# davidesantangelo/krep

Hardware: AMD Instinct MI355X
Metric: GB/s scanned (literal scan, match offsets produced), haystack resident in HBM (higher is better)
Workload: dtype u8; 1 GPU; literal8: 8-byte case-sensitive literal 'Sherlock', ~1e-4 matches/byte, offsets tracked; 32 GiB per GPU (BASELINE.json configs[1]); pattern=Sherlock, bytes_per_gpu=34359738368, matches=3436005, parallelism=contiguous shards x1, start-offset ownership, 1 RCCL all-reduce of counts

## Files before the change

include/krep_gpu_debug.h:

```cpp
#ifndef KREP_GPU_DEBUG_H
#define KREP_GPU_DEBUG_H
#include "krep_gpu.h"
#ifdef __cplusplus
extern "C" {
#endif

uint64_t krep_gpu_debug_replay_host(int krep_ref_algo, const void *text, size_t n, const void *pattern, uint32_t m,
                                    int whole_word, size_t cur, int open_line);
void krep_gpu_debug_force_rounds(int rounds);
void krep_gpu_debug_force_stage_cap(int records);
void krep_gpu_debug_force_single_grid(int blocks);
uint64_t krep_gpu_debug_single_failovers(void);
uint64_t krep_gpu_debug_single_launches(void);
uint64_t krep_gpu_debug_tiny_launches(void);
uint64_t krep_gpu_debug_tiny_dense_launches(void);
void krep_gpu_debug_inject_failure(int kind);
void krep_gpu_debug_chain_fixups(uint64_t *rescans, uint64_t *replays);
void krep_gpu_debug_fold_carry(const krep_gpu_seq_carry_t *in, const krep_gpu_seq_carry_t *piece, krep_gpu_seq_carry_t *out);
uint64_t krep_gpu_debug_anchored_launches(void);
uint64_t krep_gpu_debug_literal_dma_launches(void);
int krep_gpu_debug_literal_dma_state(const krep_gpu_plan_t *plan, int *looked, int *barred, double *pass_rate);
uint64_t krep_gpu_debug_runs_launches(void);
int krep_gpu_debug_split_state(const krep_gpu_plan_t *plan);
int krep_gpu_debug_anchor_info(const krep_gpu_plan_t *plan, int *state, uint32_t *moved, double *rate_end_grams, double *rate_anchors);
int krep_gpu_debug_anchor_measured(const krep_gpu_plan_t *plan, double *measured, int *resamples);

#ifdef __cplusplus
}
#endif
#endif
```

krep_amd/csrc/kg_config.hip:

```cpp
#include <hip/hip_runtime.h>

#include <algorithm>
#include <atomic>
#include <chrono>
#include <cstdarg>
#include <cstdio>
#include <cstdlib>
#include <cstring>
#include <mutex>
#include <string>
#include <vector>

#include "../../include/krep_gpu.h"
#include "kg_common.h"
#include "kg_internal.h"
#include "kg_plan.h"
#include "kg_replay.h"

using namespace kg;

static thread_local std::string g_err;
namespace kg {
int fail(const char *fmt, ...)
{
// ... 194 lines not shown
    const char *r = kg::device_unusable(kg::current_config().device);
    return r ? r : "";
}

namespace kg {
std::atomic<int> g_force_rounds{0};
std::atomic<int> g_force_stage_cap{0};
}
extern "C" void krep_gpu_debug_force_stage_cap(int c) { g_force_stage_cap.store(c); }
extern "C" void krep_gpu_debug_force_rounds(int r) { g_force_rounds.store(r); }
namespace kg {
extern int g_s1_force_grid;
std::atomic<uint64_t> g_fused1_failovers{0};
}
extern "C" void krep_gpu_debug_force_single_grid(int blocks) { kg::g_s1_force_grid = blocks < 0 ? 0 : blocks; }
extern "C" uint64_t krep_gpu_debug_single_failovers(void) { return g_fused1_failovers.load(); }
namespace kg {
std::atomic<uint64_t> g_fused1_launches{0};
}
extern "C" uint64_t krep_gpu_debug_single_launches(void) { return kg::g_fused1_launches.load(); }
namespace kg {
std::atomic<uint64_t> g_tiny_launches{0};
}
extern "C" uint64_t krep_gpu_debug_tiny_launches(void) { return kg::g_tiny_launches.load(); }
namespace kg {
std::atomic<uint64_t> g_tiny_dense_launches{0};
}
extern "C" uint64_t krep_gpu_debug_tiny_dense_launches(void) { return kg::g_tiny_dense_launches.load(); }
namespace kg {
std::atomic<uint64_t> g_ac_anchored_launches{0};
}
extern "C" uint64_t krep_gpu_debug_anchored_launches(void) { return kg::g_ac_anchored_launches.load(); }
extern "C" uint64_t krep_gpu_debug_literal_dma_launches(void) { return kg::g_lit_dma_launches.load(); }
extern "C" uint64_t krep_gpu_debug_runs_launches(void) { return kg::g_runs_launches.load(); }
```

krep_amd/csrc/kg_internal.h:

```cpp
#pragma once
#include <hip/hip_runtime.h>

#include <atomic>
#include <cstring>
#include <initializer_list>
#include <vector>

#include "../../include/krep_gpu.h"
#include "../../include/krep_gpu_debug.h"
#include "kg_common.h"

namespace kg {

int fail(const char *fmt, ...);
const char *device_unusable(int device);
bool inject(int kind);
#define HIPCHK(x)                                                                                 \
    do                                                                                            \
    {                                                                                             \
        hipError_t e_ = (x);                                                                      \
        if (e_ != hipSuccess)                                                                     \
            return kg::fail("%s failed: %s (%s:%d)", #x, hipGetErrorString(e_), __FILE__, __LINE__); \
    } while (0)

// ... 22 lines not shown
}

template <auto Kernel> hipError_t grant_dynamic_lds(int bytes)
{
    static std::atomic<bool> granted[64];
    int dev = 0;
    (void)hipGetDevice(&dev);
    const bool known = dev >= 0 && dev < 64;
    if (known && granted[dev].load(std::memory_order_acquire))
        return hipSuccess;
    const hipError_t e = hipFuncSetAttribute(reinterpret_cast<const void *>(Kernel), hipFuncAttributeMaxDynamicSharedMemorySize, bytes);
    if (e == hipSuccess && known)
        granted[dev].store(true, std::memory_order_release);
    return e;
}

hipError_t launch_literal(const LitArgs &a, uint32_t num_cu, hipStream_t st);
int runs_count_greedy(const uint8_t *d_text, uint64_t text_len, uint64_t lo, uint64_t hi, uint32_t m, uint8_t byte, bool ci, int num_cu,
                      unsigned long long *d_slots, unsigned long long *h_slots, hipStream_t st, uint64_t *total, uint64_t *end_p1);
bool literal_dma_eligible(const LitArgs &a);
hipError_t launch_literal_dma(const LitArgs &a, uint32_t num_cu, hipStream_t st);
hipError_t launch_dma_byte_look(const uint8_t *text, uint64_t lo, uint32_t n_cells, uint32_t prefilter, bool ci, unsigned long long *out, hipStream_t st);
extern std::atomic<uint64_t> g_runs_launches;
extern std::atomic<uint64_t> g_lit_dma_launches;

struct PostScratch;
constexpr int kFusedShapeMax = 5;
double single_fused_max_density(int shape);
int single_fused_shape_for(double density, double margin, int start);
bool single_fused_reopens(uint64_t total, uint64_t span);
constexpr int kFusedGaveUp = 1;
int single_fused_run(const LitArgs &a, uint64_t n_units, uint64_t span, PostScratch &post, Counters *d_ctr, Counters *h_ctr,
                     uint32_t num_cu, int *shape, hipEvent_t ev_end, hipStream_t st, bool count_launch);

struct PostScratch
{
    unsigned long long *d_unitinfo = nullptr;
    unsigned long long *d_offsets = nullptr;
    unsigned long long *d_blk = nullptr;
    uint64_t units_cap = 0;
    unsigned long long *d_stage = nullptr;
    uint64_t stage_cap_words = 0;
    uint64_t *d_occ = nullptr;
    uint64_t occ_cap = 0;
    uint8_t *d_keep = nullptr;
    unsigned long long *d_gblk = nullptr;
    unsigned long long *d_surv = nullptr;
    uint64_t keep_cap = 0;
    unsigned long long *d_tk = nullptr;
    uint64_t tk_cap = 0;
};
void post_free(PostScratch &s);
int post_reserve(PostScratch &s, uint64_t n_units, uint64_t stage_words);
int post_order(PostScratch &s, uint64_t n_units, uint32_t stage_cap, uint32_t fixed_len, uint64_t origin, uint64_t unit_bytes,
               bool want_lines, uint64_t *d_pos, uint64_t pos_cap, Counters *d_ctr, int num_cu, hipStream_t st);
int post_offsets_pass(PostScratch &s, uint64_t n_units, bool want_lines, Counters *d_ctr, hipStream_t st);
int post_gather_pass(PostScratch &s, uint64_t n_units, uint32_t stage_cap, uint32_t fixed_len, uint64_t origin,
                     uint64_t unit_bytes, uint64_t *d_pos, uint64_t pos_cap, int num_cu, hipStream_t st);
constexpr uint32_t kWalkGreedy = 0;
constexpr uint32_t kWalkShortO = 1;
constexpr uint32_t kWalkShortOLines = 2;
struct WalkSpec
{
    uint32_t mode, m;
    bool ww, lines, ci;
    uint8_t b1, b2;
// ... 95 lines not shown
```

krep_amd/csrc/kg_literal_dma.hip:

```cpp
#include <hip/hip_runtime.h>
#include <algorithm>
#include <atomic>
#include <cstdlib>
#include "kg_common.h"
#include "kg_device.h"
#include "kg_internal.h"

namespace kg {

namespace {

constexpr u32 kDmaPark = 80;
constexpr u32 kDmaRing = 2u * kSegBytes;
constexpr u32 kDmaTail = 256u;
constexpr u32 kDmaWaveLds = kDmaRing + kDmaTail;
}

template <int KIND, bool MASKED, bool CI>
__global__ __launch_bounds__(kBlock, 2) void lit_scan_dma(const LitArgs a)
{
    extern __shared__ __attribute__((aligned(16))) uint8_t d_smem[];
    __shared__ u64 s_info_all[kWavesPerBlk][kDmaPark];
    __shared__ __attribute__((aligned(16))) unsigned short s_slots_all[kWavesPerBlk][kDmaPark * 16u];
    __shared__ u32 s_unit_all[kWavesPerBlk][kDmaPark];
    const u32 lane = lane_id();
    const u32 wave = __builtin_amdgcn_readfirstlane(threadIdx.x >> 6);
    uint8_t *ring = d_smem + wave * kDmaWaveLds;
    uint8_t *tailb = ring + kDmaRing;
    u64 *s_info = s_info_all[wave];
    unsigned short *s_slots = s_slots_all[wave];
    u32 *s_unit = s_unit_all[wave];
    const u32 ring_lds = (u32)(size_t)(__attribute__((address_space(3))) uint8_t *)ring;

    const bool want_pos = (a.flags & F_POS) != 0;
    const bool ww = (a.flags & F_WW) != 0;
    const u64 hi_match = (a.own_hi < a.text_len - a.m + 1) ? a.own_hi : (a.text_len - a.m + 1);
    constexpr u64 kUnitBytes = (u64)kRoundsBig * kSegBytes;
    const u64 n_units = a.num_tiles * kWavesPerBlk;

    const bool park = want_pos && a.stage_cap >= 16u && a.stage_cap <= 128u && (a.stage_cap & 7u) == 0u && n_units < (1ull << 32);
    const u32 park_max = park ? kDmaPark * 16u / a.stage_cap : 0u;
    u32 n_park = 0;
    auto flush_parked = [&]() __attribute__((always_inline)) {
        for (u32 i = lane; i < n_park; i += 64u)
        {
            const u64 u = s_unit[i];
            a.unitinfo[u] = s_info[i];
            if (s_info[i] & kUiCountMask)
            {
                uint4 *dst = reinterpret_cast<uint4 *>(reinterpret_cast<unsigned short *>(a.stage) + u * (u64)a.stage_cap);
                const uint4 *src = reinterpret_cast<const uint4 *>(&s_slots[i * a.stage_cap]);
                const u32 c = (u32)(s_info[i] & kUiCountMask), nv = ((c < a.stage_cap ? c : a.stage_cap) + 7u) >> 3;
                for (u32 q = 0; q < nv; ++q)
                    dst[q] = src[q];
            }
        }
        n_park = 0;
    };

    const u32 tk_units = a.upt ? a.upt : 1u;
    u64 static_next = (u64)blockIdx.x * kWavesPerBlk + wave;
    auto next_ticket = [&]() -> u64 {
        if (a.upt)
        {
            return wave_fetch_add(&a.ctr->ticket, 1ull, lane) * (u64)a.upt;
        }
        const u64 u = static_next;
        static_next += (u64)gridDim.x * kWavesPerBlk;
        return u;
    };
    auto issue_round = [&](u64 seg, u32 buf) -> bool {
        if (seg + kSegBytes > a.text_len)
            return false;
        const uint8_t *src = a.text + seg + lane * 16u;
        uint8_t *dst = ring + buf * kSegBytes;
#pragma unroll
        for (int j = 0; j < kCells; ++j)
            __builtin_amdgcn_global_load_lds((const __attribute__((address_space(1))) void *)(src + j * kCellBytes),
                                             (__attribute__((address_space(3))) void *)(dst + j * kCellBytes), 16, 0, 2 );
        return true;
    };
    auto issue_tail = [&](u64 at) -> bool {
        if (at + kDmaTail > a.text_len)
            return false;
        __builtin_amdgcn_global_load_lds((const __attribute__((address_space(1))) void *)(a.text + at + lane * 4u),
                                         (__attribute__((address_space(3))) void *)tailb, 4, 0, 0);
        return true;
    };

    u64 acc_total = 0;
    u32 pf_cells = 0;
    u32 wcnt = 0;
    auto stage_hit = [&](u64 unit, u32 idx, u32 rel) __attribute__((always_inline)) {
        if (idx < a.stage_cap)
        {
            unsigned short *slot = park ? &s_slots[n_park * a.stage_cap] : reinterpret_cast<unsigned short *>(a.stage) + unit * (u64)a.stage_cap;
            slot[idx] = (unsigned short)rel;
        }
    };
    auto publish = [&](u64 unit) __attribute__((always_inline)) {
        acc_total += wcnt;
        if (want_pos)
        {
            if (lane == 0)
            {
                const u64 info = (u64)wcnt | (wcnt ? (kLnHead | kLnTail) : 0ull);
                if (park)
                {
                    s_info[n_park] = info;
                    s_unit[n_park] = (u32)unit;
                }
                else
                    a.unitinfo[unit] = info;
                if (wcnt > a.stage_cap)
                {
                    atomicAdd(&a.ctr->overflow_units, 1ull);
                    atomicMax(&a.ctr->max_unit_count, (u64)wcnt);
                }
            }
            if (park && ++n_park == park_max)
                flush_parked();
        }
        wcnt = 0;
    };
    auto exact = [&](u32 A0, u32 A4) -> bool {
        const u32 e0 = CI ? (A0 | a.l0) : A0;
        bool h = (KIND == 4 && MASKED) ? (((e0 ^ a.p0) & a.k0) == 0u) : (e0 == a.p0);
        if (KIND >= 8)
        {
            const u32 e4 = CI ? (A4 | a.l1) : A4;
            h = h && ((KIND == 8 && MASKED) ? (((e4 ^ a.p1) & a.k1) == 0u) : (e4 == a.p1));
        }
        return h;
    };
    auto owned = [&](u64 p) -> bool { return p >= a.own_lo && p < hi_match && !(p >= a.excl_lo && p < a.excl_hi); };
    auto word_ok = [&](u64 p) -> bool {
        if (p > 0 && p != a.ww_exempt_left && is_wordc(a.text[p - 1]))
            return false;
        if (p + a.m < a.text_len && is_wordc(a.text[p + a.m]))
            return false;
        return true;
    };
    auto boundary = [&](u64 seg_prev, u64 unit, u32 r_prev, u32 c0, u32 c1, u32 n0, u32 n1) __attribute__((always_inline)) {
        {
            const u32 f = 0x01010101u * ((CI ? (a.p0 | 0x20u) : a.p0) & 0xffu);
            const u32 y0 = (CI ? (c0 | 0x20202020u) : c0) ^ f, y1 = (CI ? (c1 | 0x20202020u) : c1) ^ f;
            if (((((y0 - 0x01010101u) & ~y0) | ((y1 - 0x01010101u) & ~y1)) & 0x80808080u) == 0u)
                return;
        }
        const u32 q = lane & 7u, sh = q & 3u;
        const bool up = (q >> 2) != 0u;
        const u32 lo = up ? c1 : c0, mid = up ? n0 : c1, hi = up ? n1 : n0;
        const u32 A0 = __builtin_amdgcn_alignbyte(mid, lo, sh), A4 = __builtin_amdgcn_alignbyte(hi, mid, sh);
        const u64 p = seg_prev + (kSegBytes - 8u) + q;
        bool h = lane < 8u && q + a.m > 8u && exact(A0, A4) && owned(p);
        if (ww && __ballot(h))
            h = h && word_ok(p);
        const u64 bm = __ballot(h);
        if (bm)
        {
            if (h && want_pos)
                stage_hit(unit, wcnt + mbcnt64(bm), r_prev * kSegBytes + (kSegBytes - 8u) + q);
            wcnt += (u32)__popcll(bm);
        }
    };

    u64 u0 = next_ticket();
    bool dma_cur = u0 < n_units && issue_round(a.anchor + u0 * kUnitBytes, 0u);
    while (u0 < n_units)
    {
        const u32 nun = (u32)((n_units - u0 < (u64)tk_units) ? (n_units - u0) : (u64)tk_units), nr = nun * (u32)kRoundsBig;
        const u64 tbase = a.anchor + u0 * kUnitBytes;
        u64 u_next = ~0ull;
        bool tail_ok = false;
        u32 c0 = 0, c1 = 0;
        bool deferred = false;
#pragma unroll 1
        for (u32 g = 0; g < nr; ++g)
        {
            const u64 seg = tbase + (u64)g * kSegBytes, unit = u0 + (g >> 2);
            const u32 r = g & 3u;
            bool dma_nx = false, tail_now = false;
            asm volatile("s_waitcnt lgkmcnt(0)" ::: "memory");
            if (g + 1u < nr)
                dma_nx = issue_round(seg + kSegBytes, (g + 1u) & 1u);
            else
            {
                u_next = next_ticket();
                if (u_next < n_units)
                    dma_nx = issue_round(a.anchor + u_next * kUnitBytes, (g + 1u) & 1u);
            }
            if (g + 2u == nr)
                tail_ok = tail_now = issue_tail(tbase + (u64)nr * kSegBytes);
            if (dma_cur)
            {
                if (dma_nx && tail_now)
                    asm volatile("s_waitcnt vmcnt(9)" ::: "memory");
                else if (dma_nx)
                    asm volatile("s_waitcnt vmcnt(8)" ::: "memory");
                else if (tail_now)
                    asm volatile("s_waitcnt vmcnt(1)" ::: "memory");
                else
                    asm volatile("s_waitcnt vmcnt(0)" ::: "memory");
            }
            const bool interior = seg >= a.own_lo && seg + kSegBytes <= hi_match && (seg + kSegBytes <= a.excl_lo || seg >= a.excl_hi);
            uint4 vv[kCells];
            uint2 nn[kCells];
            if (dma_cur)
            {
                typedef u32 v4 __attribute__((ext_vector_type(4)));
                typedef u32 v2 __attribute__((ext_vector_type(2)));
                const u32 addr = ring_lds + (g & 1u) * kSegBytes + lane * 16u;
                v4 x[kCells];
                v2 y[kCells];
#pragma unroll
                for (int j = 0; j < kCells; ++j)
                {
                    asm volatile("ds_read_b128 %0, %1 offset:%2" : "=v"(x[j]) : "v"(addr), "n"(j * (int)kCellBytes));
                    asm volatile("ds_read_b64 %0, %1 offset:%2" : "=v"(y[j]) : "v"(addr), "n"(j * (int)kCellBytes + 16));
                }
                asm volatile("s_waitcnt lgkmcnt(0)"
                             : "+v"(x[0]), "+v"(x[1]), "+v"(x[2]), "+v"(x[3]), "+v"(x[4]), "+v"(x[5]), "+v"(x[6]), "+v"(x[7]), "+v"(y[0]), "+v"(y[1]),
                               "+v"(y[2]), "+v"(y[3]), "+v"(y[4]), "+v"(y[5]), "+v"(y[6]), "+v"(y[7])
                             :
                             : "memory");
#pragma unroll
                for (int j = 0; j < kCells; ++j)
                {
                    vv[j] = make_uint4(x[j].x, x[j].y, x[j].z, x[j].w);
                    nn[j] = make_uint2(y[j].x, y[j].y);
                }
            }
            else
            {
#pragma unroll
                for (int j = 0; j < kCells; ++j)
                {
                    const W6 w = load_window_guarded(a.text, a.text_len, seg + (u64)j * kCellBytes + (u64)lane * 16u);
                    vv[j] = make_uint4(w.v[0], w.v[1], w.v[2], w.v[3]);
                    nn[j] = make_uint2(w.v[4], w.v[5]);
                }
            }
            if (deferred)
            {
                boundary(seg - kSegBytes, u0 + ((g - 1u) >> 2), (g - 1u) & 3u, c0, c1, __builtin_amdgcn_readfirstlane(vv[0].x),
                         __builtin_amdgcn_readfirstlane(vv[0].y));
                deferred = false;
                if (r == 0u)
                    publish(unit - 1u);
            }
            __builtin_amdgcn_sched_barrier(0);
#pragma unroll
            for (int j = 0; j < kCells; ++j)
            {
                const u64 lbase = seg + (u64)j * kCellBytes + (u64)lane * 16u;
                const u32 D[6] = {vv[j].x, vv[j].y, vv[j].z, vv[j].w, nn[j].x, nn[j].y};
                auto A = [&](int k) -> u32 {
                    return ((k & 3) == 0) ? D[k >> 2] : __builtin_amdgcn_alignbyte(D[(k >> 2) + 1], D[k >> 2], (u32)(k & 3));
                };
                u32 Dq[6];
#pragma unroll
                for (int w = 0; w < 6; ++w)
                    Dq[w] = CI ? (D[w] | 0x20202020u) : D[w];
                auto Aq = [&](int k) -> u32 {
                    return ((k & 3) == 0) ? Dq[k >> 2] : __builtin_amdgcn_alignbyte(Dq[(k >> 2) + 1], Dq[k >> 2], (u32)(k & 3));
                };
                const u32 p0q = CI ? (a.p0 | 0x20202020u) : a.p0;
                if (a.prefilter)
                {
                    u32 z = 0;
#pragma unroll
                    for (int w = 0; w < 4; ++w)
                    {
                        const u32 y = Dq[w] ^ a.prefilter;
                        z |= (y - 0x01010101u) & ~y;
                    }
                    if (!__ballot((z & 0x80808080u) != 0u))
                        continue;
                    ++pf_cells;
                }
                bool c[16];
                u64 any = 0;
#pragma unroll
// ... 75 lines not shown
                    }
                }
            }
            if (dma_cur)
            {
                c0 = __builtin_amdgcn_readlane(vv[kCells - 1].z, 63);
                c1 = __builtin_amdgcn_readlane(vv[kCells - 1].w, 63);
                deferred = true;
            }
            if (g + 1u == nr)
            {
                if (deferred)
                {
                    u32 n0 = 0, n1 = 0;
                    if (tail_ok)
                    {
                        typedef u32 v2 __attribute__((ext_vector_type(2)));
                        v2 t;
                        const u32 taddr = ring_lds + kDmaRing;
                        asm volatile("ds_read_b64 %0, %1\n\ts_waitcnt lgkmcnt(0)" : "=v"(t) : "v"(taddr) : "memory");
                        n0 = __builtin_amdgcn_readfirstlane(t.x);
                        n1 = __builtin_amdgcn_readfirstlane(t.y);
                    }
                    else
                    {
                        const W6 w = load_window_guarded(a.text, a.text_len, seg + kSegBytes);
                        n0 = __builtin_amdgcn_readfirstlane(w.v[0]);
                        n1 = __builtin_amdgcn_readfirstlane(w.v[1]);
                    }
                    boundary(seg, unit, r, c0, c1, n0, n1);
                    deferred = false;
                }
                publish(unit);
            }
            else if (!deferred && r == 3u)
                publish(unit);
            dma_cur = dma_nx;
        }
        u0 = u_next;
    }
    if (park && n_park)
        flush_parked();
    if (lane == 0 && acc_total)
        atomicAdd(&a.ctr->total, acc_total);
    if (lane == 0 && pf_cells)
        atomicAdd(&a.ctr->candidates, (u64)pf_cells);
}

__global__ __launch_bounds__(256) void dma_byte_look(const uint8_t *text, u64 lo, u32 n_cells, u32 b4, u32 fold, unsigned long long *out)
{
    const u32 lane = lane_id();
    const u32 wave = blockIdx.x * 4u + (threadIdx.x >> 6), n_waves = gridDim.x * 4u;
    u32 cnt = 0;
    for (u32 c = wave; c < n_cells; c += n_waves)
    {
        const uint4 v = *reinterpret_cast<const uint4 *>(text + lo + (u64)c * kCellBytes + lane * 16u);
        const u32 d[4] = {v.x, v.y, v.z, v.w};
        u32 z = 0;
#pragma unroll
        for (int w = 0; w < 4; ++w)
        {
            const u32 y = (d[w] | fold) ^ b4;
            z |= (y - 0x01010101u) & ~y;
        }
        if (__ballot((z & 0x80808080u) != 0u))
            ++cnt;
    }
    if (lane == 0 && cnt)
        atomicAdd(out, (u64)cnt);
}
hipError_t launch_dma_byte_look(const uint8_t *text, uint64_t lo, uint32_t n_cells, uint32_t prefilter, bool ci, unsigned long long *out, hipStream_t st)
{
    hipLaunchKernelGGL(dma_byte_look, dim3(256), dim3(256), 0, st, text, (u64)lo, n_cells, prefilter, ci ? 0x20202020u : 0u, out);
    return hipGetLastError();
}

std::atomic<uint64_t> g_lit_dma_launches{0};

template <int KIND, bool MASKED, bool CI>
static hipError_t dma_launch3(const LitArgs &a, u32 num_cu, hipStream_t st)
{
    constexpr u32 lds = kWavesPerBlk * kDmaWaveLds;
    if (const hipError_t e = grant_dynamic_lds<&lit_scan_dma<KIND, MASKED, CI>>((int)lds); e != hipSuccess)
        return e;
    static const u32 bpc = [] { const char *e = getenv("KREP_GPU_LIT_DMA_BLOCKS_PER_CU"); return e && atoi(e) > 0 ? (u32)atoi(e) : 2u; }();
    const u32 grid = (u32)std::min<u64>(a.num_tiles, (u64)num_cu * bpc);
    hipLaunchKernelGGL((lit_scan_dma<KIND, MASKED, CI>), dim3(grid ? grid : 1), dim3(kBlock), lds, st, a);
    g_lit_dma_launches.fetch_add(1, std::memory_order_relaxed);
    return hipGetLastError();
}
template <int KIND, bool MASKED>
static hipError_t dma_launch2(const LitArgs &a, u32 num_cu, hipStream_t st)
{
    return (a.flags & F_CI) ? dma_launch3<KIND, MASKED, true>(a, num_cu, st) : dma_launch3<KIND, MASKED, false>(a, num_cu, st);
}

bool literal_dma_eligible(const LitArgs &a)
{
    return !getenv("KREP_GPU_LIT_NO_DMA") && a.prefilter != 0u && a.m >= 2 && a.m <= 8 && a.rounds == (u32)kRoundsBig && !(a.flags & F_LINES) && !a.emit_mode &&
           (a.upt >= 4 || getenv("KREP_GPU_LIT_DMA_ALL")) && a.text_len >= 4u * kSegBytes;
}
hipError_t launch_literal_dma(const LitArgs &a, u32 num_cu, hipStream_t st)
{
    if (a.m < 4)
        return dma_launch2<4, true>(a, num_cu, st);
    if (a.m == 4)
        return dma_launch2<4, false>(a, num_cu, st);
    if (a.m < 8)
        return dma_launch2<8, true>(a, num_cu, st);
    return dma_launch2<8, false>(a, num_cu, st);
}

}
```

krep_amd/csrc/kg_plan.h:

```cpp
#pragma once
#include <hip/hip_runtime.h>

#include <vector>

#include "../../include/krep_gpu.h"
#include "kg_common.h"
#include "kg_internal.h"

struct krep_gpu_plan
{
    krep_gpu_config_t cfg{};
    int device = 0;
    int ref_algo = KREP_RA_NONE;
    const char *unsupported = nullptr;
    bool only_matching = false;
    bool cs = true, ww = false, lines = false, track = false;
    size_t max_count = SIZE_MAX;
    std::vector<std::vector<uint8_t>> pats;
    uint32_t m = 0, p0 = 0, p1 = 0, k0 = 0, k1 = 0, l0 = 0, l1 = 0;
    uint32_t p2 = 0, p3 = 0, k2 = 0, k3 = 0, l2 = 0, l3 = 0;
    std::vector<uint8_t> pat_folded;
    bool has_border = false;
    bool has_newline = false;
    uint8_t *d_pat = nullptr;
    unsigned long long *d_pat_chunks = nullptr;
    uint32_t n_chunks = 0;
    kg::Counters *d_ctr = nullptr, *h_ctr = nullptr;
    int num_cu = 256;
    hipEvent_t ev0 = nullptr, ev1 = nullptr;
    kg::AcTables *ac = nullptr;
    kg::AcTables *ac_long = nullptr, *ac_short = nullptr;
    int ac_split = 0;
    match_position_t *d_split_rec = nullptr;
    uint64_t split_cap = 0;
    bool ac_has_newline = false;
    kg::PostScratch post;
    uint32_t sparse_cap = 16;
    bool dma_look_done = false;
    bool dma_off = false;
    const void *dma_off_text = nullptr;
    size_t dma_off_len = 0;
    double dma_pass_rate = 0;
    bool first_look_done = false;
    bool fused1_ok = true;
    bool fusedk_on = false;
    bool fusedk_never = false;
    int fusedk_shape = 0;
    int fused1_shape = 0;
    match_position_t *d_nl_rec = nullptr;
    uint64_t *d_nl_ln = nullptr;
    uint64_t nl_cap = 0;
    bool lines_list_off = false;
    kg::PostScratch aux;
    search_params_t sp{};
    std::vector<const char *> pat_ptrs;
    std::vector<size_t> pat_lens;
};
namespace kg {
struct Window
{
    const uint8_t *d_text;
    size_t text_len;
    size_t own_lo, own_hi;
    size_t global_base;
    size_t global_len;
};
int stop_clock(krep_gpu_plan *pl, bool record_ev1, hipStream_t st, krep_gpu_scan_out_t *out);
int nl_reserve(krep_gpu_plan *pl, uint64_t need, uint64_t want, bool with_ln);
int scan_ac(krep_gpu_plan *pl, const Window &w, match_position_t *d_pos, uint64_t cap, hipStream_t st, int time_it,
            const krep_gpu_seq_carry_t *carry_in, krep_gpu_seq_carry_t *carry_out, krep_gpu_scan_out_t *out);
}
```

krep_amd/csrc/kg_scan.hip:

```cpp
#include <hip/hip_runtime.h>

#include <algorithm>
#include <cstdio>
#include <cstdlib>
#include <cstring>
#include <vector>

#include "../../include/krep_gpu.h"
#include "kg_common.h"
#include "kg_internal.h"
#include "kg_plan.h"
#include "kg_replay.h"

using namespace kg;

struct Verdict { uint64_t ret, store; };
static Verdict verdict_for(int algo, const krep_gpu_plan *pl, uint64_t total, uint64_t lines, bool have_result)
{
    const size_t maxc = pl->max_count;
    const bool store = pl->track && have_result;
    Verdict v{0, 0};
    switch (algo)
    {
    case KREP_RA_MEMCHR:
// ... 293 lines not shown
static void lit_learn_density(krep_gpu_plan *pl, const LitPass &ps, const LitScan &L)
{
    const LitArgs &a = L.a;
    const uint32_t m_scan = a.m;
    if ((a.flags & F_POS) && m_scan != 1 && a.rounds == kRoundsBig && pl->h_ctr->overflow_units * 64 > L.n_units && !L.fsc)
    {
        uint32_t want = 64;
        if (pl->sparse_cap >= 64)
            for (want = 128; want < 256 && want < pl->h_ctr->max_unit_count; want *= 2) {}
        pl->sparse_cap = std::max(pl->sparse_cap, want);
    }
    if ((a.flags & F_POS) && m_scan >= 2 && m_scan <= 8 && a.rounds == kRoundsBig && !L.fsc && !pl->fusedk_never &&
        ps.sink == LitPass::RECORDS && !ps.lines && L.hi_match > a.anchor)
    {
        const double density = L.density(pl->h_ctr->total);
        if (density * 32768.0 >= fusedk_min_hits_per_unit() && density <= single_fused_max_density(kFusedShapeMax))
        {
            pl->fusedk_on = true;
            pl->fusedk_shape = single_fused_shape_for(density, 1.0, 0);
        }
    }
    if (getenv("KREP_GPU_DEBUG") && (a.flags & F_POS))
        fprintf(stderr, "krep-gpu: literal scan: %llu of %llu units overflowed a %u-entry slot (fullest: %llu); one-pass next: %d (shape %d)\n",
                pl->h_ctr->overflow_units, (unsigned long long)L.n_units, a.stage_cap, pl->h_ctr->max_unit_count, (int)pl->fusedk_on,
                pl->fusedk_shape);
}
static void lit_reopen(krep_gpu_plan *pl, const LitScan &L)
{
    const uint32_t m_scan = L.a.m;
    if (!pl->fused1_ok && m_scan == 1 && single_fused_reopens(pl->h_ctr->total, L.span()))
        pl->fused1_ok = true;
    if (pl->fusedk_never && m_scan >= 2 && m_scan <= 8 && single_fused_reopens(pl->h_ctr->total, L.span()))
        pl->fusedk_never = false;
}

static int lit_two_pass(krep_gpu_plan *pl, const Window &w, const LitPass &ps, LitScan &L, bool chain, hipStream_t st)
{
    LitArgs &a = L.a;
    a.positions = ps.d_out;
    a.pos_cap = ps.sink == LitPass::RECORDS ? ps.out_cap : 0;
    HIPCHK(launch_literal(a, (uint32_t)pl->num_cu, st));
    if (chain && post_order(*ps.post, L.n_units, a.stage_cap, a.m, a.anchor + w.global_base, L.unit_bytes(), ps.lines, ps.d_out, a.pos_cap,
                            pl->d_ctr, pl->num_cu, st))
        return 2;
    if (ps.ev_end) HIPCHK(hipEventRecord(ps.ev_end, st));
    HIPCHK(hipMemcpyAsync(pl->h_ctr, pl->d_ctr, sizeof(Counters), hipMemcpyDeviceToHost, st));
    HIPCHK(hipStreamSynchronize(st));
    lit_dma_rate(pl, w, L);
    lit_learn_density(pl, ps, L);
    if ((a.flags & F_POS) && pl->h_ctr->overflow_units)
    {
        LitArgs e = a;
        e.emit_mode = 1;
        HIPCHK(hipMemsetAsync(&pl->d_ctr->ticket, 0, sizeof(unsigned long long), st));
        HIPCHK(launch_literal(e, (uint32_t)pl->num_cu, st));
        if (ps.ev_end) HIPCHK(hipEventRecord(ps.ev_end, st));
    }
    return 0;
}
static int lit_two_pass_occ(krep_gpu_plan *pl, const Window &w, const LitPass &ps, const LitScan &L, hipStream_t st)
{
    const LitArgs &a = L.a;
    PostScratch &post = *ps.post;
    HIPCHK(launch_literal(a, (uint32_t)pl->num_cu, st));
    if (post_offsets_pass(post, L.n_units, false, pl->d_ctr, st))
        return 2;
// ... 6 lines not shown
        if (post_gather_pass(post, L.n_units, a.stage_cap, a.m, a.anchor + w.global_base, L.unit_bytes(), post.d_occ, n_occ, pl->num_cu, st))
            return 2;
        if (pl->h_ctr->overflow_units)
        {
            LitArgs e = a;
            e.emit_mode = 1;
            e.positions = post.d_occ;
            e.pos_cap = n_occ;
            HIPCHK(hipMemsetAsync(&pl->d_ctr->ticket, 0, sizeof(unsigned long long), st));
            HIPCHK(launch_literal(e, (uint32_t)pl->num_cu, st));
        }
    }
    return 0;
}

static int lit_pass(krep_gpu_plan *pl, const Window &w, const LitPass &ps, hipStream_t st, LitResult *res)
{
    *res = LitResult{};
    const uint32_t m_scan = ps.first_byte ? 1u : pl->m;
    size_t own_hi = std::min(ps.own_hi, w.text_len);
    if (ps.first_byte)
        own_hi = std::min<size_t>(own_hi, w.text_len - pl->m + 1);
    const uint64_t hi_match = std::min<uint64_t>(own_hi, w.text_len - m_scan + 1);
    if (hi_match <= ps.own_lo)
        return 0;
    LitScan L = lit_args(pl, w, ps, own_hi, hi_match);
    if (lit_dma_look(pl, w, ps, L, st))
        return 2;
    res->n_units = L.n_units;
    res->unit_bytes = L.unit_bytes();
    res->anchor = L.a.anchor;
    bool done = false;
    if (lit_first_look(pl, ps, L, st) || lit_one_pass(pl, w, ps, L, st, res, &done))
        return 2;
    if (done)
        return 0;
    const bool chain = (L.a.flags & (F_POS | F_LINES)) != 0;
    if (chain)
    {
        PostScratch &post = *ps.post;
        if (post_reserve(post, L.n_units, (L.n_units * L.a.stage_cap + 3) / 4))
            return 2;
        L.a.unitinfo = post.d_unitinfo;
        L.a.stage = (uint64_t *)post.d_stage;
        L.a.offsets = (const uint64_t *)post.d_offsets;
    }
    HIPCHK(hipMemsetAsync(pl->d_ctr, 0, sizeof(Counters), st));
    if (ps.sink != LitPass::OCC ? lit_two_pass(pl, w, ps, L, chain, st) : lit_two_pass_occ(pl, w, ps, L, st))
        return 2;
    res->total = pl->h_ctr->total;
    res->lines = pl->h_ctr->lines;
    lit_reopen(pl, L);
    res->summary = chain ? pl->h_ctr->summary : (res->total ? (kLnHead | kLnTail) : 0);
    return 0;
}

namespace {
struct Family
{
    bool greedy = false;
    bool mshort_o = false;
    bool need_walk = false;
    bool replay = false;
    bool neon_zero = false;
    bool nlwalk = false;
    bool whole_text() const { return need_walk || replay || neon_zero || nlwalk; }
// ... 764 lines not shown
```

krep_amd/engine.py:

```python
from __future__ import annotations

import ctypes as C
import os

import numpy as np

from . import abi

HERE = os.path.dirname(os.path.abspath(__file__))
LIB_PATH = os.path.join(HERE, "lib", "libkrep_gpu.so")


class KrepGpuError(RuntimeError):
    pass


class Engine:

    def __init__(self, path: str = LIB_PATH):
        path = os.environ.get("KREP_GPU_LIB", path)
        if not os.path.exists(path):
            raise KrepGpuError(f"{path} is missing: build it with `python -m krep_amd.build` "
                               "(hipcc --offload-arch=gfx950); there is no CPU fallback")
        if not os.environ.get("KREP_GPU_NO_TORCH"):
# ... 74 lines not shown
        L.krep_gpu_comm_init_rank.restype = C.c_int
        L.krep_gpu_comm_init_rank.argtypes = [C.c_void_p, C.c_int, C.c_int, C.c_int]
        L.krep_gpu_comm_allreduce_u64.restype = C.c_int
        L.krep_gpu_comm_allreduce_u64.argtypes = [C.POINTER(C.c_uint64), C.c_int]
        L.krep_gpu_comm_allreduce_device_u64.restype = C.c_int
        L.krep_gpu_comm_allreduce_device_u64.argtypes = [C.c_void_p, C.c_int, C.c_void_p]
        L.krep_gpu_comm_destroy.restype = None
        L.krep_gpu_rccl_calls.restype = C.c_uint64
        L.krep_gpu_rccl_version.restype = C.c_int
        L.krep_gpu_debug_force_single_grid.restype = None
        L.krep_gpu_debug_force_single_grid.argtypes = [C.c_int]
        L.krep_gpu_debug_single_failovers.restype = C.c_uint64
        L.krep_gpu_debug_single_launches.restype = C.c_uint64
        L.krep_gpu_debug_tiny_launches.restype = C.c_uint64
        L.krep_gpu_debug_chain_fixups.restype = None
        L.krep_gpu_debug_chain_fixups.argtypes = [C.POINTER(C.c_uint64), C.POINTER(C.c_uint64)]
        L.krep_gpu_debug_tiny_dense_launches.restype = C.c_uint64
        if hasattr(L, "krep_gpu_debug_anchor_info"):
            L.krep_gpu_debug_anchored_launches.restype = C.c_uint64
            L.krep_gpu_debug_literal_dma_launches.restype = C.c_uint64
            L.krep_gpu_debug_runs_launches.restype = C.c_uint64
            L.krep_gpu_debug_anchor_info.restype = C.c_int
            L.krep_gpu_debug_anchor_info.argtypes = [C.c_void_p, C.POINTER(C.c_int), C.POINTER(C.c_uint32), C.POINTER(C.c_double),
                                                     C.POINTER(C.c_double)]
        if hasattr(L, "krep_gpu_alloc_placed"):
            L.krep_gpu_alloc_placed.restype = C.c_int
            L.krep_gpu_alloc_placed.argtypes = [C.c_int, C.c_size_t, C.c_size_t, C.c_int, C.POINTER(C.c_void_p), C.POINTER(C.c_void_p),
                                                C.POINTER(abi.Placement)]
            L.krep_gpu_free_placed.restype = C.c_int
            L.krep_gpu_free_placed.argtypes = [C.c_int, C.c_void_p]
        if hasattr(L, "krep_gpu_debug_literal_dma_state"):
            L.krep_gpu_debug_literal_dma_state.restype = C.c_int
            L.krep_gpu_debug_literal_dma_state.argtypes = [C.c_void_p, C.POINTER(C.c_int), C.POINTER(C.c_int), C.POINTER(C.c_double)]
        if hasattr(L, "krep_gpu_debug_anchor_measured"):
            L.krep_gpu_debug_anchor_measured.restype = C.c_int
            L.krep_gpu_debug_anchor_measured.argtypes = [C.c_void_p, C.POINTER(C.c_double), C.POINTER(C.c_int)]
        L.krep_gpu_last_shard_info.restype = None
        L.krep_gpu_last_shard_info.argtypes = [C.POINTER(abi.ShardInfo)]
        L.krep_gpu_available.restype = C.c_int
        L.krep_gpu_unavailable_reason.restype = C.c_char_p
        L.krep_gpu_last_status.restype = C.c_int
        L.krep_gpu_set_cpu_fallback.restype = None
        L.krep_gpu_set_cpu_fallback.argtypes = [C.c_void_p]
        L.krep_gpu_worthwhile.restype = C.c_int
        L.krep_gpu_worthwhile.argtypes = [C.POINTER(abi.SearchParams), C.c_size_t]
        L.krep_gpu_worthwhile_ex.restype = C.c_int
        L.krep_gpu_worthwhile_ex.argtypes = [C.POINTER(abi.SearchParams), C.c_size_t, C.c_int]
        L.krep_gpu_cost_estimate.restype = C.c_int
        L.krep_gpu_cost_estimate.argtypes = [C.POINTER(abi.SearchParams), C.c_size_t, C.c_int, C.POINTER(abi.Cost)]
        L.krep_gpu_get_cost_rates.restype = None
        L.krep_gpu_get_cost_rates.argtypes = [C.POINTER(abi.CostRates)]
        L.krep_gpu_set_cost_rates.restype = None
        L.krep_gpu_set_cost_rates.argtypes = [C.POINTER(abi.CostRates)]
        L.krep_gpu_set_min_text_bytes.restype = None
        L.krep_gpu_set_min_text_bytes.argtypes = [C.c_size_t]
        L.krep_gpu_device_count.restype = C.c_int
        L.krep_gpu_last_error.restype = C.c_char_p
        L.krep_gpu_clear_error.restype = None
        L.krep_gpu_version.restype = C.c_char_p

    def set_reference_simd(self, level: int):
        self.lib.krep_gpu_set_reference_simd(level)

    def set_only_matching(self, on: bool):
        self.lib.krep_gpu_set_only_matching(int(on))

    def set_force_no_simd(self, on: bool):
        self.lib.krep_gpu_set_force_no_simd(int(on))

    def set_algo_override(self, a: int):
        self.lib.krep_gpu_set_algo_override(a)

    def force_rounds(self, r: int):
        self.lib.krep_gpu_debug_force_rounds(r)

    def force_single_grid(self, blocks: int):
        self.lib.krep_gpu_debug_force_single_grid(blocks)

    def single_failovers(self) -> int:
        return int(self.lib.krep_gpu_debug_single_failovers())

    def single_launches(self) -> int:
        return int(self.lib.krep_gpu_debug_single_launches())

    def chain_fixups(self):
        a, b = C.c_uint64(0), C.c_uint64(0)
        self.lib.krep_gpu_debug_chain_fixups(C.byref(a), C.byref(b))
        return int(a.value), int(b.value)

    def tiny_dense_launches(self) -> int:
        return int(self.lib.krep_gpu_debug_tiny_dense_launches())

    def runs_launches(self) -> int:
        return int(self.lib.krep_gpu_debug_runs_launches())

    def literal_dma_launches(self) -> int:
        return int(self.lib.krep_gpu_debug_literal_dma_launches())

    def alloc_placed(self, text_bytes: int, record_bytes: int, tries: int = 3, device: int = 0):
        t, r, info = C.c_void_p(0), C.c_void_p(0), abi.Placement()
        if self.lib.krep_gpu_alloc_placed(device, text_bytes, record_bytes, tries, C.byref(t), C.byref(r), C.byref(info)):
            raise KrepGpuError("krep_gpu_alloc_placed failed: " + self.last_error())
        return int(t.value), int(r.value or 0), info

    def free_placed(self, d_text: int, device: int = 0):
        if self.lib.krep_gpu_free_placed(device, C.c_void_p(d_text)):
            raise KrepGpuError("krep_gpu_free_placed failed: " + self.last_error())

    def anchored_launches(self) -> int:
        return int(self.lib.krep_gpu_debug_anchored_launches())

    def tiny_launches(self) -> int:
        return int(self.lib.krep_gpu_debug_tiny_launches())

    def force_stage_cap(self, c: int):
        self.lib.krep_gpu_debug_force_stage_cap(c)

    def default_config(self) -> abi.Config:
        c = abi.Config()
        self.lib.krep_gpu_config_default(C.byref(c))
        return c

    def set_thread_config(self, cfg: "abi.Config | None"):
        self.lib.krep_gpu_set_thread_config(C.byref(cfg) if cfg is not None else None)

    def set_stream_chunk(self, nbytes: int):
        self.lib.krep_gpu_set_stream_chunk(nbytes)

    def can_accelerate(self, params: abi.Params) -> bool:
        return bool(self.lib.krep_gpu_can_accelerate(params.ref))

# ... 240 lines not shown
```

Baseline: 6591 GB/s.

## Add one-pass LDS-DMA literal scan with ticket decoupled-lookback offset emission

```diff
diff --git a/include/krep_gpu_debug.h b/include/krep_gpu_debug.h
--- a/include/krep_gpu_debug.h
+++ b/include/krep_gpu_debug.h
@@ -20,6 +20,8 @@
 uint64_t krep_gpu_debug_anchored_launches(void);
 uint64_t krep_gpu_debug_literal_dma_launches(void);
 int krep_gpu_debug_literal_dma_state(const krep_gpu_plan_t *plan, int *looked, int *barred, double *pass_rate);
+void krep_gpu_debug_force_dma_grid(int blocks);
+void krep_gpu_debug_literal_dma_one_pass(uint64_t *launches, uint64_t *failovers);
 uint64_t krep_gpu_debug_runs_launches(void);
 int krep_gpu_debug_split_state(const krep_gpu_plan_t *plan);
 int krep_gpu_debug_anchor_info(const krep_gpu_plan_t *plan, int *state, uint32_t *moved, double *rate_end_grams, double *rate_anchors);
diff --git a/krep_amd/csrc/kg_config.hip b/krep_amd/csrc/kg_config.hip
--- a/krep_amd/csrc/kg_config.hip
+++ b/krep_amd/csrc/kg_config.hip
@@ -250,4 +250,13 @@
 }
 extern "C" uint64_t krep_gpu_debug_anchored_launches(void) { return kg::g_ac_anchored_launches.load(); }
 extern "C" uint64_t krep_gpu_debug_literal_dma_launches(void) { return kg::g_lit_dma_launches.load(); }
+namespace kg {
+std::atomic<uint64_t> g_lit_dma1_launches{0}, g_lit_dma1_failovers{0};
+}
+extern "C" void krep_gpu_debug_force_dma_grid(int blocks) { kg::g_dma_force_grid = blocks < 0 ? 0 : blocks; }
+extern "C" void krep_gpu_debug_literal_dma_one_pass(uint64_t *launches, uint64_t *failovers)
+{
+    if (launches) *launches = kg::g_lit_dma1_launches.load();
+    if (failovers) *failovers = kg::g_lit_dma1_failovers.load();
+}
 extern "C" uint64_t krep_gpu_debug_runs_launches(void) { return kg::g_runs_launches.load(); }
diff --git a/krep_amd/csrc/kg_internal.h b/krep_amd/csrc/kg_internal.h
--- a/krep_amd/csrc/kg_internal.h
+++ b/krep_amd/csrc/kg_internal.h
@@ -78,6 +78,10 @@
 constexpr int kFusedGaveUp = 1;
 int single_fused_run(const LitArgs &a, uint64_t n_units, uint64_t span, PostScratch &post, Counters *d_ctr, Counters *h_ctr,
                      uint32_t num_cu, int *shape, hipEvent_t ev_end, hipStream_t st, bool count_launch);
+int literal_dma_one_pass(const LitArgs &a, PostScratch &post, Counters *d_ctr, Counters *h_ctr, uint32_t num_cu, hipEvent_t ev_end, hipStream_t st);
+uint32_t literal_dma_one_pass_ring();
+extern int g_dma_force_grid;
+extern std::atomic<uint64_t> g_lit_dma1_launches, g_lit_dma1_failovers;
 
 struct PostScratch
 {
diff --git a/krep_amd/csrc/kg_literal_dma.hip b/krep_amd/csrc/kg_literal_dma.hip
--- a/krep_amd/csrc/kg_literal_dma.hip
+++ b/krep_amd/csrc/kg_literal_dma.hip
@@ -5,6 +5,7 @@
 #include "kg_common.h"
 #include "kg_device.h"
 #include "kg_internal.h"
+#include "kg_tickets.h"
 
 namespace kg {
 
@@ -14,17 +15,36 @@
 constexpr u32 kDmaRing = 2u * kSegBytes;
 constexpr u32 kDmaTail = 256u;
 constexpr u32 kDmaWaveLds = kDmaRing + kDmaTail;
-}
-
-template <int KIND, bool MASKED, bool CI>
-__global__ __launch_bounds__(kBlock, 2) void lit_scan_dma(const LitArgs a)
+constexpr u32 kDmaRecHalf = 448u;
+}
+
+template <int KIND, bool MASKED, bool CI, bool ONE>
+__global__ __launch_bounds__(kBlock, 2) void lit_scan_dma(const LitArgs a, u64 *__restrict__ agg, u64 *__restrict__ pref, const u64 n_tickets)
 {
     extern __shared__ __attribute__((aligned(16))) uint8_t d_smem[];
-    __shared__ u64 s_info_all[kWavesPerBlk][kDmaPark];
-    __shared__ __attribute__((aligned(16))) unsigned short s_slots_all[kWavesPerBlk][kDmaPark * 16u];
-    __shared__ u32 s_unit_all[kWavesPerBlk][kDmaPark];
+    __shared__ u64 s_info_all[kWavesPerBlk][ONE ? 1u : kDmaPark];
+    __shared__ __attribute__((aligned(16))) unsigned short s_slots_all[kWavesPerBlk][ONE ? 8u : kDmaPark * 16u];
+    __shared__ u32 s_unit_all[kWavesPerBlk][ONE ? 1u : kDmaPark];
+    __shared__ u32 s_rec_all[kWavesPerBlk][ONE ? 2u * kDmaRecHalf : 1u];
     const u32 lane = lane_id();
     const u32 wave = __builtin_amdgcn_readfirstlane(threadIdx.x >> 6);
+    if constexpr (ONE)
+    {
+        bool resolver = false;
+        if (wave == 0)
+        {
+            u64 r = 1;
+            if (lane == 0)
+                r = __hip_atomic_fetch_add(&a.ctr->pad[0], 1ull, __ATOMIC_RELAXED, __HIP_MEMORY_SCOPE_AGENT);
+            resolver = rfl64(r) == 0ull;
+        }
+        if (resolver)
+        {
+            tk_resolve(agg, pref, n_tickets, a.ctr, lane);
+            return;
+        }
+    }
+    u32 *s_rec = s_rec_all[wave];
     uint8_t *ring = d_smem + wave * kDmaWaveLds;
     uint8_t *tailb = ring + kDmaRing;
     u64 *s_info = s_info_all[wave];
@@ -38,7 +58,7 @@
     constexpr u64 kUnitBytes = (u64)kRoundsBig * kSegBytes;
     const u64 n_units = a.num_tiles * kWavesPerBlk;
 
-    const bool park = want_pos && a.stage_cap >= 16u && a.stage_cap <= 128u && (a.stage_cap & 7u) == 0u && n_units < (1ull << 32);
+    const bool park = !ONE && want_pos && a.stage_cap >= 16u && a.stage_cap <= 128u && (a.stage_cap & 7u) == 0u && n_units < (1ull << 32);
     const u32 park_max = park ? kDmaPark * 16u / a.stage_cap : 0u;
     u32 n_park = 0;
     auto flush_parked = [&]() __attribute__((always_inline)) {
@@ -60,10 +80,12 @@
 
     const u32 tk_units = a.upt ? a.upt : 1u;
     u64 static_next = (u64)blockIdx.x * kWavesPerBlk + wave;
+    u64 t_drawn = 0;
     auto next_ticket = [&]() -> u64 {
         if (a.upt)
         {
-            return wave_fetch_add(&a.ctr->ticket, 1ull, lane) * (u64)a.upt;
+            t_drawn = wave_fetch_add(&a.ctr->ticket, 1ull, lane);
+            return t_drawn * (u64)a.upt;
         }
         const u64 u = static_next;
         static_next += (u64)gridDim.x * kWavesPerBlk;
@@ -91,14 +113,31 @@
     u64 acc_total = 0;
     u32 pf_cells = 0;
     u32 wcnt = 0;
+    u64 t_cur = 0, u0 = 0;
+    u32 tk_cnt = 0, half = 0;
+    bool pend = false, nxt = false, overflowed = false;
+    u64 pend_t = 0, pend_base = 0, pref_pre = 0, nxt_t = 0, nxt_base = 0;
+    u32 pend_half = 0, pend_cnt = 0, nxt_half = 0, nxt_cnt = 0;
     auto stage_hit = [&](u64 unit, u32 idx, u32 rel) __attribute__((always_inline)) {
-        if (idx < a.stage_cap)
+        if constexpr (ONE)
+        {
+            const u32 i = tk_cnt + idx;
+            if (i < kDmaRecHalf)
+                s_rec[half * kDmaRecHalf + i] = (u32)(unit - u0) * (u32)kUnitBytes + rel;
+        }
+        else if (idx < a.stage_cap)
         {
             unsigned short *slot = park ? &s_slots[n_park * a.stage_cap] : reinterpret_cast<unsigned short *>(a.stage) + unit * (u64)a.stage_cap;
             slot[idx] = (unsigned short)rel;
         }
     };
     auto publish = [&](u64 unit) __attribute__((always_inline)) {
+        if constexpr (ONE)
+        {
+            tk_cnt += wcnt;
+            wcnt = 0;
+            return;
+        }
         acc_total += wcnt;
         if (want_pos)
         {
@@ -122,6 +161,56 @@
                 flush_parked();
         }
         wcnt = 0;
+    };
+    auto flush = [&]() __attribute__((always_inline)) {
+        const u64 first = (pref_pre & kTkReady) ? (pref_pre & ~kTkReady) : tk_wait_prefix(pref, pend_t, a.ctr, lane);
+        const u32 pad = (u32)(first & 7ull);
+        const u32 *src = s_rec + pend_half * kDmaRecHalf;
+        for (u32 g = lane; g < pend_cnt + pad; g += 64u)
+        {
+            if (g < pad)
+                continue;
+            const u32 i = g - pad;
+            const u64 idx = first + i;
+            if (idx < a.pos_cap)
+            {
+                const u64 st = pend_base + src[i], en = st + a.m;
+                typedef u32 u32x4 __attribute__((ext_vector_type(4)));
+                const u32x4 rec = {(u32)st, (u32)(st >> 32), (u32)en, (u32)(en >> 32)};
+                __builtin_nontemporal_store(rec, reinterpret_cast<u32x4 *>(a.positions + 2 * idx));
+            }
+        }
+        pend = false;
+        pref_pre = 0;
+    };
+    auto ticket_done = [&](u64 tbase) __attribute__((always_inline)) {
+        if (tk_cnt > kDmaRecHalf)
+            overflowed = true;
+        if (lane == 0)
+            __hip_atomic_store(&agg[t_cur], (u64)tk_cnt | kTkReady, __ATOMIC_RELAXED, __HIP_MEMORY_SCOPE_AGENT);
+        if (tk_cnt && tk_cnt <= kDmaRecHalf)
+        {
+            nxt = true;
+            nxt_t = t_cur;
+            nxt_base = tbase + a.global_base;
+            nxt_half = half;
+            nxt_cnt = tk_cnt;
+            half ^= 1u;
+        }
+        tk_cnt = 0;
+    };
+    auto rotate = [&]() __attribute__((always_inline)) {
+        if (pend)
+            flush();
+        if (nxt)
+        {
+            pend = true;
+            pend_t = nxt_t;
+            pend_base = nxt_base;
+            pend_half = nxt_half;
+            pend_cnt = nxt_cnt;
+            nxt = false;
+        }
     };
     auto exact = [&](u32 A0, u32 A4) -> bool {
         const u32 e0 = CI ? (A0 | a.l0) : A0;
@@ -165,7 +254,8 @@
         }
     };
 
-    u64 u0 = next_ticket();
+    u0 = next_ticket();
+    t_cur = t_drawn;
     bool dma_cur = u0 < n_units && issue_round(a.anchor + u0 * kUnitBytes, 0u);
     while (u0 < n_units)
     {
@@ -186,7 +276,16 @@
                 dma_nx = issue_round(seg + kSegBytes, (g + 1u) & 1u);
             else
             {
+                if (ONE && pend)
+                {
+                    u64 pp = 0;
+                    if (lane == 0)
+                        pp = __hip_atomic_load(&pref[pend_t], __ATOMIC_RELAXED, __HIP_MEMORY_SCOPE_AGENT);
+                    pref_pre = pp;
+                }
                 u_next = next_ticket();
+                if (ONE)
+                    pref_pre = rfl64(pref_pre);
                 if (u_next < n_units)
                     dma_nx = issue_round(a.anchor + u_next * kUnitBytes, (g + 1u) & 1u);
             }
@@ -249,6 +348,9 @@
                 if (r == 0u)
                     publish(unit - 1u);
             }
+            if constexpr (ONE)
+                if (g == 0u)
+                    rotate();
             __builtin_amdgcn_sched_barrier(0);
 #pragma unroll
             for (int j = 0; j < kCells; ++j)
@@ -390,15 +492,26 @@
                     deferred = false;
                 }
                 publish(unit);
+                if constexpr (ONE)
+                    ticket_done(tbase);
             }
             else if (!deferred && r == 3u)
                 publish(unit);
             dma_cur = dma_nx;
         }
         u0 = u_next;
+        t_cur = t_drawn;
     }
     if (park && n_park)
         flush_parked();
+    if constexpr (ONE)
+    {
+        rotate();
+        if (pend)
+            flush();
+        if (overflowed && lane == 0)
+            atomicAdd(&a.ctr->overflow_units, 1ull);
+    }
     if (lane == 0 && acc_total)
         atomicAdd(&a.ctr->total, acc_total);
     if (lane == 0 && pf_cells)
@@ -434,23 +547,38 @@
 }
 
 std::atomic<uint64_t> g_lit_dma_launches{0};
-
-template <int KIND, bool MASKED, bool CI>
-static hipError_t dma_launch3(const LitArgs &a, u32 num_cu, hipStream_t st)
+int g_dma_force_grid = 0;
+
+template <int KIND, bool MASKED, bool CI, bool ONE>
+static hipError_t dma_launch3(const LitArgs &a, u64 *agg, u64 *pref, u64 n_tickets, u32 num_cu, hipStream_t st)
 {
     constexpr u32 lds = kWavesPerBlk * kDmaWaveLds;
-    if (const hipError_t e = grant_dynamic_lds<&lit_scan_dma<KIND, MASKED, CI>>((int)lds); e != hipSuccess)
+    if (const hipError_t e = grant_dynamic_lds<&lit_scan_dma<KIND, MASKED, CI, ONE>>((int)lds); e != hipSuccess)
         return e;
     static const u32 bpc = [] { const char *e = getenv("KREP_GPU_LIT_DMA_BLOCKS_PER_CU"); return e && atoi(e) > 0 ? (u32)atoi(e) : 2u; }();
-    const u32 grid = (u32)std::min<u64>(a.num_tiles, (u64)num_cu * bpc);
-    hipLaunchKernelGGL((lit_scan_dma<KIND, MASKED, CI>), dim3(grid ? grid : 1), dim3(kBlock), lds, st, a);
+    u32 grid = (u32)std::min<u64>(a.num_tiles, (u64)num_cu * bpc);
+    if (g_dma_force_grid > 0)
+        grid = std::min<u32>(grid, (u32)g_dma_force_grid);
+    hipLaunchKernelGGL((lit_scan_dma<KIND, MASKED, CI, ONE>), dim3(grid ? grid : 1), dim3(kBlock), lds, st, a, agg, pref, n_tickets);
     g_lit_dma_launches.fetch_add(1, std::memory_order_relaxed);
     return hipGetLastError();
 }
-template <int KIND, bool MASKED>
-static hipError_t dma_launch2(const LitArgs &a, u32 num_cu, hipStream_t st)
-{
-    return (a.flags & F_CI) ? dma_launch3<KIND, MASKED, true>(a, num_cu, st) : dma_launch3<KIND, MASKED, false>(a, num_cu, st);
+template <int KIND, bool MASKED, bool ONE>
+static hipError_t dma_launch2(const LitArgs &a, u64 *agg, u64 *pref, u64 n_tickets, u32 num_cu, hipStream_t st)
+{
+    return (a.flags & F_CI) ? dma_launch3<KIND, MASKED, true, ONE>(a, agg, pref, n_tickets, num_cu, st)
+                            : dma_launch3<KIND, MASKED, false, ONE>(a, agg, pref, n_tickets, num_cu, st);
+}
+template <bool ONE>
+static hipError_t dma_launch(const LitArgs &a, u64 *agg, u64 *pref, u64 n_tickets, u32 num_cu, hipStream_t st)
+{
+    if (a.m < 4)
+        return dma_launch2<4, true, ONE>(a, agg, pref, n_tickets, num_cu, st);
+    if (a.m == 4)
+        return dma_launch2<4, false, ONE>(a, agg, pref, n_tickets, num_cu, st);
+    if (a.m < 8)
+        return dma_launch2<8, true, ONE>(a, agg, pref, n_tickets, num_cu, st);
+    return dma_launch2<8, false, ONE>(a, agg, pref, n_tickets, num_cu, st);
 }
 
 bool literal_dma_eligible(const LitArgs &a)
@@ -458,15 +586,24 @@
     return !getenv("KREP_GPU_LIT_NO_DMA") && a.prefilter != 0u && a.m >= 2 && a.m <= 8 && a.rounds == (u32)kRoundsBig && !(a.flags & F_LINES) && !a.emit_mode &&
            (a.upt >= 4 || getenv("KREP_GPU_LIT_DMA_ALL")) && a.text_len >= 4u * kSegBytes;
 }
-hipError_t launch_literal_dma(const LitArgs &a, u32 num_cu, hipStream_t st)
-{
-    if (a.m < 4)
-        return dma_launch2<4, true>(a, num_cu, st);
-    if (a.m == 4)
-        return dma_launch2<4, false>(a, num_cu, st);
-    if (a.m < 8)
-        return dma_launch2<8, true>(a, num_cu, st);
-    return dma_launch2<8, false>(a, num_cu, st);
-}
-
-}
+hipError_t launch_literal_dma(const LitArgs &a, u32 num_cu, hipStream_t st) { return dma_launch<false>(a, nullptr, nullptr, 0, num_cu, st); }
+
+uint32_t literal_dma_one_pass_ring() { return kDmaRecHalf; }
+uint64_t literal_dma_one_pass_tickets(const LitArgs &a) { return a.upt ? (a.num_tiles * kWavesPerBlk + a.upt - 1) / a.upt : 0; }
+int literal_dma_one_pass(const LitArgs &a, PostScratch &post, Counters *d_ctr, Counters *h_ctr, u32 num_cu, hipEvent_t ev_end, hipStream_t st)
+{
+    if (!a.upt || !(a.flags & F_POS) || (a.flags & F_LINES) || a.emit_mode || a.excl_lo != a.excl_hi)
+        return kFusedGaveUp;
+    const uint64_t n_tk = literal_dma_one_pass_tickets(a);
+    const size_t tk_bytes = 2 * n_tk * sizeof(unsigned long long);
+    HIPCHK(grow_scratch(post.tk_cap, n_tk, n_tk, {dev_buf(post.d_tk, tk_bytes)}));
+    HIPCHK(hipMemsetAsync(d_ctr, 0, sizeof(Counters), st));
+    HIPCHK(hipMemsetAsync(post.d_tk, 0, tk_bytes, st));
+    HIPCHK(dma_launch<true>(a, post.d_tk, post.d_tk + n_tk, n_tk, num_cu, st));
+    if (ev_end) HIPCHK(hipEventRecord(ev_end, st));
+    HIPCHK(hipMemcpyAsync(h_ctr, d_ctr, sizeof(Counters), hipMemcpyDeviceToHost, st));
+    HIPCHK(hipStreamSynchronize(st));
+    return h_ctr->overflow_units ? kFusedGaveUp : 0;
+}
+
+}
diff --git a/krep_amd/csrc/kg_plan.h b/krep_amd/csrc/kg_plan.h
--- a/krep_amd/csrc/kg_plan.h
+++ b/krep_amd/csrc/kg_plan.h
@@ -41,6 +41,9 @@
     const void *dma_off_text = nullptr;
     size_t dma_off_len = 0;
     double dma_pass_rate = 0;
+    bool dma1_never = false;
+    const void *dma1_never_text = nullptr;
+    size_t dma1_never_len = 0;
     bool first_look_done = false;
     bool fused1_ok = true;
     bool fusedk_on = false;
diff --git a/krep_amd/csrc/kg_scan.hip b/krep_amd/csrc/kg_scan.hip
--- a/krep_amd/csrc/kg_scan.hip
+++ b/krep_amd/csrc/kg_scan.hip
@@ -349,6 +349,40 @@
         pl->fused1_ok = true;
     if (pl->fusedk_never && m_scan >= 2 && m_scan <= 8 && single_fused_reopens(pl->h_ctr->total, L.span()))
         pl->fusedk_never = false;
+    if (pl->dma1_never && (pl->dma1_never_text != (const void *)L.a.text || pl->dma1_never_len != L.a.text_len) && L.a.upt &&
+        L.density(pl->h_ctr->total) * (double)L.a.upt * (double)L.unit_bytes() < 0.25 * (double)literal_dma_one_pass_ring())
+        pl->dma1_never = false;
+}
+
+static int lit_dma_one_pass(krep_gpu_plan *pl, const Window &w, const LitPass &ps, LitScan &L, hipStream_t st, LitResult *res, bool *done)
+{
+    LitArgs &a = L.a;
+    *done = false;
+    if (!(literal_dma_eligible(a) && a.upt > 0 && ps.sink == LitPass::RECORDS && !ps.lines && !ps.first_byte && ps.excl_lo == ps.excl_hi &&
+          L.fsc == 0 && !pl->dma1_never && !getenv("KREP_GPU_LIT_DMA_TWO_PASS")))
+        return 0;
+    a.positions = ps.d_out;
+    a.pos_cap = ps.out_cap;
+    g_lit_dma1_launches.fetch_add(1);
+    const int rc = literal_dma_one_pass(a, *ps.post, pl->d_ctr, pl->h_ctr, (uint32_t)pl->num_cu, ps.ev_end, st);
+    if (rc == 2)
+        return 2;
+    lit_dma_rate(pl, w, L);
+    if (rc != kFusedGaveUp)
+    {
+        res->total = pl->h_ctr->total;
+        res->summary = res->total ? (kLnHead | kLnTail) : 0;
+        lit_learn_density(pl, ps, L);
+        *done = true;
+        return 0;
+    }
+    pl->dma1_never = true;
+    pl->dma1_never_text = w.d_text;
+    pl->dma1_never_len = w.text_len;
+    g_lit_dma1_failovers.fetch_add(1);
+    if (getenv("KREP_GPU_DEBUG"))
+        fprintf(stderr, "krep-gpu: literal scan: a ticket overflowed the one-pass ring of the LDS-DMA kernel -> the two-pass road\n");
+    return 0;
 }
 
 static int lit_two_pass(krep_gpu_plan *pl, const Window &w, const LitPass &ps, LitScan &L, bool chain, hipStream_t st)
@@ -421,6 +455,8 @@
     res->anchor = L.a.anchor;
     bool done = false;
     if (lit_first_look(pl, ps, L, st) || lit_one_pass(pl, w, ps, L, st, res, &done))
+        return 2;
+    if (!done && lit_dma_one_pass(pl, w, ps, L, st, res, &done))
         return 2;
     if (done)
         return 0;
diff --git a/krep_amd/engine.py b/krep_amd/engine.py
--- a/krep_amd/engine.py
+++ b/krep_amd/engine.py
@@ -130,6 +130,11 @@
         if hasattr(L, "krep_gpu_debug_literal_dma_state"):
             L.krep_gpu_debug_literal_dma_state.restype = C.c_int
             L.krep_gpu_debug_literal_dma_state.argtypes = [C.c_void_p, C.POINTER(C.c_int), C.POINTER(C.c_int), C.POINTER(C.c_double)]
+        if hasattr(L, "krep_gpu_debug_force_dma_grid"):
+            L.krep_gpu_debug_force_dma_grid.restype = None
+            L.krep_gpu_debug_force_dma_grid.argtypes = [C.c_int]
+            L.krep_gpu_debug_literal_dma_one_pass.restype = None
+            L.krep_gpu_debug_literal_dma_one_pass.argtypes = [C.POINTER(C.c_uint64), C.POINTER(C.c_uint64)]
         if hasattr(L, "krep_gpu_debug_anchor_measured"):
             L.krep_gpu_debug_anchor_measured.restype = C.c_int
             L.krep_gpu_debug_anchor_measured.argtypes = [C.c_void_p, C.POINTER(C.c_double), C.POINTER(C.c_int)]
@@ -195,6 +200,14 @@
     def literal_dma_launches(self) -> int:
         return int(self.lib.krep_gpu_debug_literal_dma_launches())
 
+    def force_dma_grid(self, blocks: int):
+        self.lib.krep_gpu_debug_force_dma_grid(blocks)
+
+    def literal_dma_one_pass(self):
+        a, b = C.c_uint64(0), C.c_uint64(0)
+        self.lib.krep_gpu_debug_literal_dma_one_pass(C.byref(a), C.byref(b))
+        return int(a.value), int(b.value)
+
     def alloc_placed(self, text_bytes: int, record_bytes: int, tries: int = 3, device: int = 0):
         t, r, info = C.c_void_p(0), C.c_void_p(0), abi.Placement()
         if self.lib.krep_gpu_alloc_placed(device, text_bytes, record_bytes, tries, C.byref(t), C.byref(r), C.byref(info)):
```

Result: no change. 6612 GB/s, median of 6 (+0.3%).
